# chan0park/node2vec-by-ecc

Hardware: AMD Instinct MI355X
Metric: walk-steps/s (higher is better)
Workload: dtype f64 alias draw / int32 ids (walk); f32 (SGNS)

## Files before the change

### node2vec-by-ecc_amd/csrc/n2v_tables.hip

```cpp
#include "n2v_walk_step.h"
#include "n2v_wave_table.h"

namespace {

using n2v::uni;
using n2v::uni64;

constexpr int kLdsSlots = 512;

struct TabArgs {
    n2v::RowCtx g;
    const int32_t* src_of;
    const int64_t* edge_off;
    const int32_t* order;
    int64_t e_begin, e_end;
    const n2v_edge_rec* recs;
    n2v_alias_slot* thin;
    n2v_fat_slot* fat;
    int32_t* status;
    unsigned long long* work;
    unsigned char* scratch;
    int64_t max_k;
};

constexpr int kChunk = 16;

template <typename Slot>
__device__ __forceinline__ void emit_fat(const TabArgs& a, const Slot* T, int64_t t0, int64_t base, int K, int lane) {
    for (int k = lane; k < K; k += 64) {
        const double q = T[k].q;
        const int J = T[k].J;
        n2v::write_fat_slot(a.fat + t0 + k, q, a.recs + base + k, a.recs + base + J);
    }
}

struct FatEmit {
    const n2v_edge_rec* recs;
    n2v_fat_slot* fat;
    __device__ __forceinline__ void operator()(bool active, int idx, double q, int J) const {
        if (active) n2v::write_fat_slot(fat + idx, q, recs + idx, recs + J);
    }
};
struct ThinEmit {
    n2v_alias_slot* thin;
    __device__ __forceinline__ void operator()(bool active, int idx, double q, int J) const {
        if (!active) return;
        n2v_alias_slot s;
        s.q = q; s.J = J; s.aux = 0;
        thin[idx] = s;
    }
};

template <bool FAT, int RULE>
__global__ void __launch_bounds__(256) edge_tables_wave_kernel(TabArgs a) {
    __shared__ n2v_alias_slot lds[4 * kLdsSlots];
    __shared__ double feed[4 * n2v::kFeed];
    __shared__ int32_t rows[4 * n2v::kRowCache];
    const int lane = threadIdx.x & 63;
    const int wv = __builtin_amdgcn_readfirstlane(threadIdx.x >> 6);
    n2v_alias_slot* Tl = lds + wv * kLdsSlots;
    int32_t* my_row = rows + wv * n2v::kRowCache;
    n2v::WaveScratch ws{feed + wv * n2v::kFeed, my_row, -1};
    int32_t cached_src = -1;
    const int64_t n_waves = (int64_t)gridDim.x * 4;
    bool zero = false;
    unsigned long long nxt = 0, stat = ((unsigned long long)blockIdx.x * 4 + wv) * kChunk;
    auto request_chunk = [&]() {
        if (a.work) { if (lane == 0) nxt = atomicAdd(a.work, (unsigned long long)kChunk); }
        else { nxt = stat; stat += (unsigned long long)n_waves * kChunk; }
    };
    request_chunk();
    for (;;) {
        const int64_t i0 = a.e_begin + uni64((int64_t)nxt);
        if (i0 >= a.e_end) break;
        request_chunk();
        const int n_in = (int)min((int64_t)kChunk, a.e_end - i0);
        int32_t h_src = 0, h_dst = 0, h_K = 0;
        int64_t h_base = 0, h_t0 = 0;
        if (lane < n_in) {
            const int64_t e = a.order ? (int64_t)(uint32_t)a.order[i0 + lane] : i0 + lane;
            h_src = a.src_of[e];
            h_dst = a.g.col[e];
            h_base = a.g.row_ptr[h_dst];
            h_K = (int32_t)(a.g.row_ptr[h_dst + 1] - h_base);
            h_t0 = a.edge_off[e];
        }
      for (int j = 0; j < n_in; ++j) {
        const int32_t src = __builtin_amdgcn_readlane(h_src, j);
        const int K = __builtin_amdgcn_readlane(h_K, j);
        if (K == 0) continue;
        const int64_t base = ((int64_t)__builtin_amdgcn_readlane((int)(h_base >> 32), j) << 32) |
                             (uint32_t)__builtin_amdgcn_readlane((int)h_base, j);
        const int64_t t0 = ((int64_t)__builtin_amdgcn_readlane((int)(h_t0 >> 32), j) << 32) |
                           (uint32_t)__builtin_amdgcn_readlane((int)h_t0, j);
        if (RULE == n2v::kRuleNone && src != cached_src) {
            ws.row_n = n2v::wave_cache_row(a.g, my_row, src, lane);
            cached_src = src;
        }
        if (K <= kLdsSlots) {
            if (!n2v::wave_build_table<RULE>(a.g, Tl, ws, src, base, K, lane)) { zero = true; continue; }
            if (FAT) emit_fat(a, Tl, t0, base, K, lane);
            else for (int k = lane; k < K; k += 64) { n2v_alias_slot s = Tl[k]; s.aux = 0; a.thin[t0 + k] = s; }
            __builtin_amdgcn_wave_barrier();
        } else {
            unsigned char* row = a.scratch + ((int64_t)blockIdx.x * 4 + wv) * a.max_k * 12;
            const n2v::StreamStacks S{reinterpret_cast<int32_t*>(row + a.max_k * 8), reinterpret_cast<double*>(row)};
            int32_t* qi = reinterpret_cast<int32_t*>(Tl);
            bool ok;
            if (FAT) {
                n2v::QueueSink<FatEmit> sink{qi, qi + 128, reinterpret_cast<double*>(qi + 256), FatEmit{a.recs + base, a.fat + t0}, lane};
                ok = n2v::wave_build_stream<RULE>(a.g, S, ws, sink, src, base, K, lane);
            } else {
                n2v::QueueSink<ThinEmit> sink{qi, qi + 128, reinterpret_cast<double*>(qi + 256), ThinEmit{a.thin + t0}, lane};
                ok = n2v::wave_build_stream<RULE>(a.g, S, ws, sink, src, base, K, lane);
            }
            if (!ok) { zero = true; continue; }
            __builtin_amdgcn_wave_barrier();
        }
      }
    }
    if (zero && lane == 0) atomicOr(a.status, RULE == n2v::kRulePop ? N2V_STATUS_ZERO_POP : N2V_STATUS_ZERO_NORM);
}

}

namespace {
constexpr int kWgPerCu = n2v::wg_per_cu(4 * (kLdsSlots * 16 + n2v::kFeed * 8 + n2v::kRowCache * 4));
constexpr int64_t kMaxBlocks = 256 * kWgPerCu;
static_assert(kLdsSlots * 16 >= 2048, "the output queue of the large tables overlays the LDS table slice");
inline int64_t scratch_k(int64_t max_degree) { return max_degree <= kLdsSlots ? 0 : (max_degree + 15) / 16 * 16; }
}

extern "C" int64_t n2v_edge_tables_wave_scratch_bytes(int64_t max_degree) {
    return max_degree < 0 ? -1 : kMaxBlocks * 4 * scratch_k(max_degree) * 12;
}

namespace {
template <int RULE>
int launch_edge_tables(int64_t n_nodes, const int64_t* row_ptr, const int32_t* col, const double* w,
                       const int32_t* src_of, double p, double q, int32_t symmetric,
                       const int64_t* edge_off, const int32_t* order, int64_t e_begin, int64_t e_end,
                       const n2v_edge_rec* recs, n2v_alias_slot* thin, n2v_fat_slot* fat,
                       int32_t* status, uint64_t* work_counter, int64_t max_degree, void* scratch,
                       int64_t scratch_bytes, void* stream) {
    if (n_nodes < 0 || e_begin < 0 || e_end < e_begin || max_degree < 0)
        return n2v::fail(N2V_ERR_INVALID, "n2v_build_edge_tables_wave: bad range [%lld, %lld)", (long long)e_begin, (long long)e_end);
    if (e_end == e_begin) return N2V_OK;
    if (!row_ptr || !col || !src_of || !edge_off || !status)
        return n2v::fail(N2V_ERR_INVALID, "n2v_build_edge_tables_wave: null pointer");
    if ((thin == nullptr) == (fat == nullptr))
        return n2v::fail(N2V_ERR_INVALID, "n2v_build_edge_tables_wave: exactly one of thin / fat output");
    if (fat && !recs) return n2v::fail(N2V_ERR_INVALID, "n2v_build_edge_tables_wave: fat output needs the edge records");
    if (fat && ((uintptr_t)fat & 31) != 0) return n2v::fail(N2V_ERR_INVALID, "n2v_build_edge_tables_wave: fat slots not 32-byte aligned");
    if (!(p == p) || !(q == q)) return n2v::fail(N2V_ERR_INVALID, "n2v_build_edge_tables_wave: p or q is NaN");
    int64_t blocks = (e_end - e_begin + 4 * kChunk - 1) / (4 * kChunk);
    if (blocks > kMaxBlocks) blocks = kMaxBlocks;
    const int64_t need = blocks * 4 * scratch_k(max_degree) * 12;
    if (need > 0 && (!scratch || scratch_bytes < need || ((uintptr_t)scratch & 63) != 0))
        return n2v::fail(N2V_ERR_INVALID, "n2v_build_edge_tables_wave: max degree %lld needs %lld bytes of 64-byte aligned scratch "
                         "for %lld workgroups, got %lld", (long long)max_degree, (long long)need, (long long)blocks, (long long)scratch_bytes);
    TabArgs a{n2v::RowCtx{row_ptr, col, w, p, q, symmetric, nullptr}, src_of, edge_off, order, e_begin, e_end, recs, thin, fat, status,
              reinterpret_cast<unsigned long long*>(work_counter), reinterpret_cast<unsigned char*>(scratch), scratch_k(max_degree)};
    if constexpr (RULE == n2v::kRuleNone) {
        if (fat) {
            hipLaunchKernelGGL((edge_tables_wave_kernel<true, RULE>), dim3((unsigned)blocks), dim3(256), 0, (hipStream_t)stream, a);
            return n2v::check_launch("n2v_build_edge_tables_wave");
        }
    }
    hipLaunchKernelGGL((edge_tables_wave_kernel<false, RULE>), dim3((unsigned)blocks), dim3(256), 0, (hipStream_t)stream, a);
    return n2v::check_launch("n2v_build_edge_tables_wave");
}
}

extern "C" int n2v_build_edge_tables_wave(int64_t n_nodes, const int64_t* row_ptr, const int32_t* col, const double* w,
                                          const int32_t* src_of, double p, double q, int32_t symmetric,
                                          const int64_t* edge_off, const int32_t* order, int64_t e_begin, int64_t e_end,
                                          const n2v_edge_rec* recs, n2v_alias_slot* thin, n2v_fat_slot* fat,
                                          int32_t* status, uint64_t* work_counter, int64_t max_degree, void* scratch,
                                          int64_t scratch_bytes, void* stream) {
    return launch_edge_tables<n2v::kRuleNone>(n_nodes, row_ptr, col, w, src_of, p, q, symmetric, edge_off, order, e_begin, e_end, recs,
                                              thin, fat, status, work_counter, max_degree, scratch, scratch_bytes, stream);
}

extern "C" int n2v_build_edge_tables_wave_pop(int64_t n_nodes, const int64_t* row_ptr, const int32_t* col, const double* w,
                                              const int32_t* src_of, double p, const int64_t* edge_off, const int32_t* order,
                                              int64_t e_begin, int64_t e_end, n2v_alias_slot* thin, int32_t* status,
                                              int64_t max_degree, void* scratch, int64_t scratch_bytes, void* stream) {
    if (!thin) return n2v::fail(N2V_ERR_INVALID, "n2v_build_edge_tables_wave_pop: null output");
    if (p == 0.0) return n2v::fail(N2V_ERR_INVALID, "n2v_build_edge_tables_wave_pop: p must be non-zero");
    return launch_edge_tables<n2v::kRulePop>(n_nodes, row_ptr, col, w, src_of, p, 1.0, 0, edge_off, order, e_begin, e_end, nullptr,
                                             thin, nullptr, status, nullptr, max_degree, scratch, scratch_bytes, stream);
}
```

### node2vec-by-ecc_amd/csrc/n2v_wave_table.h

```cpp
#pragma once
#include "n2v_common.h"

namespace n2v {

__device__ __forceinline__ void wave_sync() {
    __builtin_amdgcn_fence(__ATOMIC_RELEASE, "workgroup");
    __builtin_amdgcn_wave_barrier();
    __builtin_amdgcn_fence(__ATOMIC_ACQUIRE, "workgroup");
}
__device__ __forceinline__ double unid(double v) {
    return __hiloint2double(uni(__double2hiint(v)), uni(__double2loint(v)));
}
__device__ __forceinline__ double readlane_f64(double v, int j) {
    const int lo = __builtin_amdgcn_readlane(__double2loint(v), j);
    const int hi = __builtin_amdgcn_readlane(__double2hiint(v), j);
    return __hiloint2double(hi, lo);
}

struct RowCtx {
    const int64_t* row_ptr;
    const int32_t* col;
    const double* w;
    double p, q;
    int32_t symmetric;
    const uint8_t* plain;
};

enum : int { kRuleNone = 0, kRulePop = 1 };
template <int RULE>
__device__ __forceinline__ bool norm_fails(double norm) {
    return RULE == kRulePop ? (norm == 0.0 || norm != norm) : norm == 0.0;
}

constexpr int kFeed = 64;
constexpr int kRowCache = 384;
struct WaveScratch {
    double* feed;
    const int32_t* row;
    int row_n;
    int plain_row = 0;
};

__device__ __forceinline__ int wave_cache_row(const RowCtx& a, int32_t* ws_row, int32_t src, int lane, int cap = kRowCache) {
    if (src < 0 || !a.symmetric) return -1;
    const int64_t b = uni64(a.row_ptr[src]);
    const int S = uni((int)(a.row_ptr[src + 1] - b));
    if (S > cap) return -1;
    for (int i = lane; i < S; i += 64) ws_row[i] = a.col[b + i];
    wave_sync();
    return S;
}

__device__ __forceinline__ bool lds_row_contains(const int32_t* row, int n, int32_t v) {
    int lo = 0, hi = n;
    while (lo < hi) {
        const int mid = (lo + hi) >> 1;
        if (row[mid] < v) lo = mid + 1;
        else hi = mid;
    }
    return lo < n && row[lo] == v;
}

template <int RULE>
__device__ __forceinline__ double step_weight_of(const RowCtx& a, const WaveScratch& ws, int32_t src, int32_t nb, double wt) {
    if (RULE == kRulePop) {
        if (src < 0 && ws.plain_row) return wt;
        const int64_t pop = a.row_ptr[nb + 1] - a.row_ptr[nb];
        if (pop == 0) return __longlong_as_double(0x7FF8000000000000LL);
        if (src >= 0 && nb == src) return wt / (a.p * (double)pop);
        return wt / (double)pop;
    }
    if (src < 0) return wt;
    if (nb == src) return wt / a.p;
    const bool adj = ws.row_n >= 0 ? lds_row_contains(ws.row, ws.row_n, nb)
                     : a.symmetric ? row_contains(a.row_ptr, a.col, src, nb) : row_contains(a.row_ptr, a.col, nb, src);
    return adj ? wt : wt / a.q;
}
template <int RULE>
__device__ __forceinline__ double step_weight(const RowCtx& a, const WaveScratch& ws, int32_t src, int64_t base, int k) {
    return step_weight_of<RULE>(a, ws, src, a.col[base + k], a.w ? a.w[base + k] : 1.0);
}

__device__ __forceinline__ double wave_sum_in_order(const WaveScratch& ws, double norm, double v, int cnt, int lane) {
    ws.feed[lane] = v;
    wave_sync();
    int j = 0;
    for (; j + 8 <= cnt; j += 8) {
#pragma unroll
        for (int i = 0; i < 8; ++i) norm = norm + ws.feed[j + i];
    }
    for (; j < cnt; ++j) norm = norm + ws.feed[j];
    wave_sync();
    return norm;
}

template <typename Stacks, typename Sink>
__device__ __forceinline__ void wave_pair(const Stacks& S, Sink& out, int K, int ns, int nl, int lane) {
    int mem_s = ns, mem_l = nl;
    int s_pos = 0, s_cnt = 0, l_pos = 0, l_cnt = 0;
    int si = 0, li = 0;
    double sq = 0.0, lq = 0.0;
    bool carried = false;
    int cs_i = 0;
    double cs_q = 0.0;
    for (;;) {
        if (l_pos == l_cnt) {
            if (mem_l == 0) break;
            const int pos = K - mem_l + lane;
            l_cnt = min(64, mem_l);
            if (lane < l_cnt) S.load_large(pos, li, lq);
            mem_l -= l_cnt;
            l_pos = 0;
        }
        const int large = __builtin_amdgcn_readlane(li, l_pos);
        double ql = readlane_f64(lq, l_pos);
        ++l_pos;
        if (carried) {
            out.one(cs_i, cs_q, large);
            carried = false;
            ql = ql + cs_q;
            ql = ql - 1.0;
            if (ql < 1.0) { carried = true; cs_i = large; cs_q = ql; continue; }
        }
        bool dry = false;
        for (;;) {
            if (s_pos == s_cnt) {
                if (mem_s == 0) { dry = true; break; }
                const int pos = mem_s - 1 - lane;
                s_cnt = min(64, mem_s);
                if (lane < s_cnt) S.load_small(pos, si, sq);
                mem_s -= s_cnt;
                s_pos = 0;
            }
            const int first = s_pos;
            int dem;
            {
                const int sq_lo = __double2loint(sq), sq_hi = __double2hiint(sq);
                int pos = uni(s_pos);
                const int cnt = uni(s_cnt);
                asm volatile(
                    "s_nop 3\n\t"
                    "1:\n\t"
                    "v_readlane_b32 vcc_lo, %[qlo], %[pos]\n\t"
                    "v_readlane_b32 vcc_hi, %[qhi], %[pos]\n\t"
                    "s_add_i32 %[pos], %[pos], 1\n\t"
                    "s_nop 0\n\t"
                    "v_add_f64 %[ql], %[ql], vcc\n\t"
                    "v_add_f64 %[ql], %[ql], -1.0\n\t"
                    "v_cmp_gt_f64 vcc, 1.0, %[ql]\n\t"
                    "s_cbranch_vccnz 2f\n\t"
                    "s_cmp_lt_i32 %[pos], %[cnt]\n\t"
                    "s_cbranch_scc1 1b\n\t"
                    "s_mov_b32 %[dem], 0\n\t"
                    "s_branch 3f\n\t"
                    "2:\n\t"
                    "s_mov_b32 %[dem], 1\n\t"
                    "3:\n\t"
                    : [ql] "+v"(ql), [pos] "+s"(pos), [dem] "=s"(dem)
                    : [qlo] "v"(sq_lo), [qhi] "v"(sq_hi), [cnt] "s"(cnt)
                    : "vcc", "scc");
                s_pos = pos;
            }
            const bool demoted = dem != 0;
            out.run(lane >= first && lane < s_pos, si, sq, large);
            if (demoted) { carried = true; cs_i = large; cs_q = ql; break; }
        }
        if (dry) {
            out.one(large, ql, 0);
            break;
        }
    }
    if (carried) out.one(cs_i, cs_q, 0);
    if (Sink::kRest) {
        out.rest(lane >= s_pos && lane < s_cnt, si, sq);
        while (mem_s > 0) {
            const int pos = mem_s - 1 - lane;
            const int cnt = min(64, mem_s);
            if (lane < cnt) S.load_small(pos, si, sq);
            out.rest(lane < cnt, si, sq);
            mem_s -= cnt;
        }
        out.rest(lane >= l_pos && lane < l_cnt, li, lq);
        while (mem_l > 0) {
            const int pos = K - mem_l + lane;
            const int cnt = min(64, mem_l);
            if (lane < cnt) S.load_large(pos, li, lq);
            out.rest(lane < cnt, li, lq);
            mem_l -= cnt;
        }
    }
}

template <typename Slot>
struct AosTable {
    Slot* T;
    __device__ __forceinline__ void load_small(int pos, int& idx, double& q) const { idx = T[pos].aux; q = T[idx].q; }
    __device__ __forceinline__ void load_large(int pos, int& idx, double& q) const { idx = T[pos].aux; q = T[idx].q; }
};
template <typename Slot>
struct AosSink {
    static constexpr bool kRest = false;
    Slot* T;
    int lane;
    __device__ __forceinline__ void run(bool in_run, int idx, double, int J) const { if (in_run) T[idx].J = J; }
    __device__ __forceinline__ void one(int idx, double q, int J) const { if (lane == 0) { T[idx].q = q; T[idx].J = J; } }
    __device__ __forceinline__ void rest(bool, int, double) const {}
};

template <int RULE, typename Slot>
__device__ __forceinline__ bool wave_build_table(const RowCtx& a, Slot* T, const WaveScratch ws, int32_t src, int64_t base,
                                                 int K, int lane) {
    for (int k = lane; k < K; k += 64) T[k].q = step_weight<RULE>(a, ws, src, base, k);
    wave_sync();
    double norm = 0.0;
    for (int c = 0; c < K; c += 64)
        norm = wave_sum_in_order(ws, norm, (c + lane < K) ? T[c + lane].q : 0.0, min(64, K - c), lane);
    norm = unid(norm);
    if (norm_fails<RULE>(norm)) return false;
    const double Kd = (double)K;
    int ns = 0, nl = 0;
    for (int c = 0; c < K; c += 64) {
        const int k = c + lane;
        const bool valid = k < K;
        double qk = 0.0;
        if (valid) {
            qk = Kd * (T[k].q / norm);
            T[k].q = qk;
            T[k].J = 0;
        }
        const bool is_small = valid && (qk < 1.0);
        const unsigned long long ms = __ballot(is_small), ml = __ballot(valid && !is_small);
        const unsigned long long below = (1ULL << lane) - 1ULL;
        if (is_small) T[ns + __popcll(ms & below)].aux = k;
        else if (valid) T[K - (nl + __popcll(ml & below) + 1)].aux = k;
        ns += __popcll(ms);
        nl += __popcll(ml);
    }
    ns = uni(ns);
    nl = uni(nl);
    wave_sync();
    AosSink<Slot> sink{T, lane};
    wave_pair(AosTable<Slot>{T}, sink, K, ns, nl, lane);
    wave_sync();
    return true;
}

template <int RULE, typename Slot>
__device__ __forceinline__ bool wave_weights_and_norm(const RowCtx& a, Slot* T, const WaveScratch ws, int32_t src, int64_t base,
                                                      int K, int lane, double& norm_out) {
    for (int k = lane; k < K; k += 64) T[k].q = step_weight<RULE>(a, ws, src, base, k);
    wave_sync();
    double norm = 0.0;
    for (int c = 0; c < K; c += 64)
        norm = wave_sum_in_order(ws, norm, (c + lane < K) ? T[c + lane].q : 0.0, min(64, K - c), lane);
    norm_out = unid(norm);
    return !norm_fails<RULE>(norm_out);
}
template <typename Slot>
__device__ __forceinline__ void wave_finish_table(Slot* T, int K, double norm, int lane) {
    const double Kd = (double)K;
    int ns = 0, nl = 0;
    for (int c = 0; c < K; c += 64) {
        const int k = c + lane;
        const bool valid = k < K;
        double qk = 0.0;
        if (valid) {
            qk = Kd * (T[k].q / norm);
            T[k].q = qk;
            T[k].J = 0;
        }
        const bool is_small = valid && (qk < 1.0);
        const unsigned long long ms = __ballot(is_small), ml = __ballot(valid && !is_small);
        const unsigned long long below = (1ULL << lane) - 1ULL;
        if (is_small) T[ns + __popcll(ms & below)].aux = k;
        else if (valid) T[K - (nl + __popcll(ml & below) + 1)].aux = k;
        ns += __popcll(ms);
        nl += __popcll(ml);
    }
    ns = uni(ns);
    nl = uni(nl);
    wave_sync();
    AosSink<Slot> sink{T, lane};
    wave_pair(AosTable<Slot>{T}, sink, K, ns, nl, lane);
    wave_sync();
}

struct StagedRow {
    const int32_t* g;
    const int32_t* big;
    int n, stride, n_big;
    __device__ __forceinline__ int find(int32_t v) const {
        int lo = 0, hi = n_big;
        while (lo < hi) {
            const int mid = (lo + hi) >> 1;
            if (big[mid] < v) lo = mid + 1;
            else hi = mid;
        }
        if (lo < n_big && big[lo] == v) return lo * stride;
        if (stride == 1 || lo == 0) return -1;
        const int top = min(lo * stride, n);
        int glo = (lo - 1) * stride + 1, ghi = top;
        while (glo < ghi) {
            const int mid = (glo + ghi) >> 1;
            if (g[mid] < v) glo = mid + 1;
            else ghi = mid;
        }
        return (glo < top && g[glo] == v) ? glo : -1;
    }
    __device__ __forceinline__ bool contains(int32_t v) const { return find(v) >= 0; }
};
__device__ __forceinline__ StagedRow stage_row(const int32_t* __restrict__ g, int n, int32_t* big, int cap, int lane) {
    const int stride = (n + cap - 1) / cap;
    const int n_big = (n + stride - 1) / stride;
    for (int i = lane; i < n_big; i += 64) big[i] = g[(int64_t)i * stride];
    wave_sync();
    return StagedRow{g, big, n, stride, n_big};
}

constexpr int kSpecCap = 128;
struct ClassSweep {
    const int32_t* M;
    int m;
    int smask;
    double qv;
    __device__ __forceinline__ bool sm(int cl) const { return (smask >> cl) & 1; }
    __device__ __forceinline__ double qc(int cl) const { return readlane_f64(qv, uni(cl)); }
};
struct RunIter {
    int j, top;
    int want;
    int r_top, r_cnt, r_cls;
    __device__ __forceinline__ void next(const ClassSweep& c) {
        for (;;) {
            if (top < 0) { r_cnt = 0; return; }
            const int e = j >= 0 ? uni(c.M[j]) : -4;
            const int spos = e >> 2;
            if (spos == top) {
                --j;
                r_top = top; r_cnt = 1; r_cls = e & 3;
                --top;
            } else {
                r_top = top; r_cnt = top - spos; r_cls = 0;
                top = spos;
            }
            if ((int)c.sm(r_cls) == want) return;
        }
    }
    __device__ __forceinline__ void take(const ClassSweep& c, int n) {
        r_top -= n;
        r_cnt -= n;
        if (r_cnt == 0) next(c);
    }
};
__device__ __forceinline__ int dyadic_draw(const RowCtx& a, const WaveScratch& ws, int32_t prev, int64_t base, int K, int kk,
                                           double u2, double wp, double wq, bool exact_sum, int32_t* big, int cap, int32_t* spec,
                                           int lane) {
    if (prev < 0) {
        const double q = (double)K * (1.0 / (double)K);
        return (u2 < q) ? kk : 0;
    }
    const int64_t pb = uni64(a.row_ptr[prev]);
    const int S = uni((int)(a.row_ptr[prev + 1] - pb));
    const int32_t* rc = a.col + base;
    const int32_t* rp = a.col + pb;
    const bool cached = ws.row_n >= 0;
    int n_adj = 0, p_idx = -1;
    const unsigned long long below = (1ULL << lane) - 1ULL;
    auto note = [&](bool adj, int pos) {
        const unsigned long long m = __ballot(adj);
        const int at = n_adj + __popcll(m & below);
        if (adj && at < kSpecCap) spec[at] = pos;
        n_adj += __popcll(m);
    };
    if ((cached && K <= 8 * S) || K <= S) {
        StagedRow R{rp, ws.row, S, 1, S};
        if (!cached) R = stage_row(rp, S, big, cap, lane);
        for (int c = 0; c < K; c += 64) {
            const int k = c + lane;
            bool adj = false, isp = false;
            if (k < K) {
                const int32_t nb = rc[k];
                isp = nb == prev;
                adj = !isp && R.contains(nb);
            }
            note(adj, k);
            const unsigned long long mp = __ballot(isp);
            if (mp != 0ULL) p_idx = c + __builtin_ctzll(mp);
        }
    } else {
        const StagedRow R = stage_row(rc, K, big, cap, lane);
        for (int c = 0; c < S; c += 64) {
            const int i = c + lane;
            int pos = -1;
            if (i < S) {
                const int32_t x = cached ? ws.row[i] : rp[i];
                if (x != prev) pos = R.find(x);
            }
            note(pos >= 0, pos);
        }
        p_idx = R.find(prev);
    }
    n_adj = uni(n_adj);
    p_idx = uni(p_idx);
    wave_sync();
    const int n_prev = p_idx >= 0 ? 1 : 0;
    const int m = n_adj + n_prev;
    if (m > kSpecCap) return -2;
    {
        const int v0 = lane < n_adj ? spec[lane] : 0x3FFFFFFF, v1 = 64 + lane < n_adj ? spec[64 + lane] : 0x3FFFFFFF;
        const int before = __popcll(__ballot(v0 < p_idx)) + __popcll(__ballot(v1 < p_idx));
        wave_sync();
        if (lane < n_adj) spec[lane + ((n_prev && v0 > p_idx) ? 1 : 0)] = v0 * 4 + 1;
        if (64 + lane < n_adj) spec[64 + lane + ((n_prev && v1 > p_idx) ? 1 : 0)] = v1 * 4 + 1;
        if (n_prev && lane == 0) spec[before] = p_idx * 4 + 2;
        wave_sync();
    }
    double norm;
    if (exact_sum) {
        norm = ((double)n_prev * wp + (double)n_adj) + (double)(K - n_prev - n_adj) * wq;
    } else {
        norm = 0.0;
        int pos = 0;
        for (int j = 0; j <= m; ++j) {
            const int e = j < m ? uni(spec[j]) : K * 4;
            for (int g = (e >> 2) - pos; g > 0; --g) norm = norm + wq;
            if (j < m) norm = norm + ((e & 3) == 2 ? wp : 1.0);
            pos = (e >> 2) + 1;
        }
        norm = unid(norm);
    }
    if (norm == 0.0) return -2;
    const double Kd = (double)K;
    const double q0 = Kd * (wq / norm), q1 = Kd * (1.0 / norm), q2 = Kd * (wp / norm);
    const ClassSweep c{spec, m, (q0 < 1.0 ? 1 : 0) | (q1 < 1.0 ? 2 : 0) | (q2 < 1.0 ? 4 : 0),
                       lane == 0 ? q0 : (lane == 1 ? q1 : q2)};
    int cls_kk = 0;
    {
        const int e0 = lane < m ? spec[lane] : -4, e1 = 64 + lane < m ? spec[64 + lane] : -4;
        const unsigned long long h0 = __ballot((e0 >> 2) == kk), h1 = __ballot((e1 >> 2) == kk);
        if (h0) cls_kk = __builtin_amdgcn_readlane(e0, __builtin_ctzll(h0)) & 3;
        else if (h1) cls_kk = __builtin_amdgcn_readlane(e1, __builtin_ctzll(h1)) & 3;
    }
    double q_kk = c.qc(cls_kk);
    if (q_kk < 1.0 && u2 < q_kk) return kk;
    RunIter sm_{m - 1, K - 1, 1, 0, 0, 0}, lg_{m - 1, K - 1, 0, 0, 0, 0};
    sm_.next(c);
    lg_.next(c);
    int J_kk = 0, c_i = 0;
    bool carried = false, done = false;
    double c_q = 0.0;
    while (!done && lg_.r_cnt > 0 && (carried || sm_.r_cnt > 0)) {
        const int large = lg_.r_top;
        double ql = c.qc(lg_.r_cls);
        lg_.take(c, 1);
        for (;;) {
            if (carried) {
                carried = false;
                if (c_i == kk) { J_kk = large; q_kk = c_q; done = true; break; }
                ql = ql + c_q;
                ql = ql - 1.0;
            } else {
                if (sm_.r_cnt == 0) { if (large == kk) q_kk = ql; done = true; break; }
                const double qs = c.qc(sm_.r_cls);
                int n = sm_.r_cnt;
                const bool hit = kk <= sm_.r_top && kk > sm_.r_top - n;
                if (hit) n = sm_.r_top - kk;
                int used = 0;
                bool dem = false;
                while (used < n) {
                    ql = ql + qs;
                    ql = ql - 1.0;
                    ++used;
                    if (uni((int)(ql < 1.0))) { dem = true; break; }
                }
                sm_.take(c, used);
                if (!dem) {
                    if (hit) { J_kk = large; q_kk = qs; done = true; break; }
                    continue;
                }
            }
            if (uni((int)(ql < 1.0))) {
                if (lg_.r_cnt == 0) { if (large == kk) q_kk = ql; done = true; }
                else { carried = true; c_i = large; c_q = ql; }
                break;
            }
        }
    }
    return (u2 < q_kk) ? kk : J_kk;
}

template <int RULE>
__device__ __forceinline__ int wave_draw_le64(const RowCtx& a, const WaveScratch& ws, int32_t src, int64_t base, int32_t nb, int K,
                                              int kk, double u2, bool exact_sum, double wp, double wq, int lane) {
    const bool valid = lane < K;
    double w, norm, w_kk;
    if (RULE == kRuleNone && exact_sum) {
        const bool isp = valid && src >= 0 && nb == src;
        const bool adj = valid && src >= 0 && !isp &&
                         (ws.row_n >= 0 ? lds_row_contains(ws.row, ws.row_n, nb) : row_contains(a.row_ptr, a.col, src, nb));
        const unsigned long long mp = __ballot(isp), ma = __ballot(adj);
        if (src < 0) { norm = (double)K; w_kk = 1.0; w = 1.0; }
        else {
            const int n_prev = __popcll(mp), n_adj = __popcll(ma);
            norm = ((double)n_prev * wp + (double)n_adj) + (double)(K - n_prev - n_adj) * wq;
            w_kk = ((mp >> kk) & 1ULL) ? wp : (((ma >> kk) & 1ULL) ? 1.0 : wq);
            w = isp ? wp : (adj ? 1.0 : wq);
        }
    } else {
        w = valid ? step_weight_of<RULE>(a, ws, src, nb, a.w ? a.w[base + lane] : 1.0) : 0.0;
        norm = unid(wave_sum_in_order(ws, 0.0, w, K, lane));
        if (norm_fails<RULE>(norm)) return -1;
        w_kk = readlane_f64(w, kk);
    }
    double q_kk = (double)K * (w_kk / norm);
    if (q_kk < 1.0 && u2 < q_kk) return kk;
    const double q = valid ? (double)K * (w / norm) : 0.0;
    unsigned long long ms = __ballot(valid && q < 1.0), ml = __ballot(valid && !(q < 1.0));
    int J_kk = 0;
    bool carried = false, done = false;
    int c_i = 0;
    double c_q = 0.0;
    while (!done && ml != 0ULL && (carried || ms != 0ULL)) {
        const int large = 63 - __builtin_clzll(ml);
        ml &= ~(1ULL << large);
        double ql = readlane_f64(q, large);
        for (;;) {
            int small;
            double qs;
            if (carried) { small = c_i; qs = c_q; carried = false; }
            else if (ms != 0ULL) { small = 63 - __builtin_clzll(ms); ms &= ~(1ULL << small); qs = readlane_f64(q, small); }
            else {
                if (large == kk) q_kk = ql;
                done = true;
                break;
            }
            if (small == kk) { J_kk = large; q_kk = qs; done = true; break; }
            ql = ql + qs;
            ql = ql - 1.0;
            if (uni((int)(ql < 1.0))) {
                if (ml == 0ULL) { if (large == kk) q_kk = ql; done = true; }
                else { carried = true; c_i = large; c_q = ql; }
                break;
            }
            if (large == kk && ms == 0ULL) { q_kk = ql; done = true; break; }
        }
    }
    return (u2 < q_kk) ? kk : J_kk;
}

struct StreamStacks {
    int32_t* idx;
    double* q;
    __device__ __forceinline__ void load_small(int pos, int& i, double& v) const { i = idx[pos]; v = q[pos]; }
    __device__ __forceinline__ void load_large(int pos, int& i, double& v) const { i = idx[pos]; v = q[pos]; }
};

template <typename Emit>
struct QueueSink {
    static constexpr bool kRest = true;
    int32_t* qi;
    int32_t* qJ;
    double* qq;
    Emit emit;
    int lane;
    int n = 0;
    __device__ __forceinline__ void flush64() {
        wave_sync();
        emit(true, qi[lane], qq[lane], qJ[lane]);
        wave_sync();
        const int rem = n - 64;
        if (lane < rem) { const int i = qi[64 + lane], J = qJ[64 + lane]; const double q = qq[64 + lane];
                          qi[lane] = i; qJ[lane] = J; qq[lane] = q; }
        n = rem;
    }
    __device__ __forceinline__ void run(bool in_run, int idx, double q, int J) {
        const unsigned long long m = __ballot(in_run);
        if (in_run) { const int p = n + __popcll(m & ((1ULL << lane) - 1ULL)); qi[p] = idx; qJ[p] = J; qq[p] = q; }
        n += __popcll(m);
        if (n >= 64) flush64();
    }
    __device__ __forceinline__ void one(int idx, double q, int J) {
        if (lane == 0) { qi[n] = idx; qJ[n] = J; qq[n] = q; }
        if (++n >= 64) flush64();
    }
    __device__ __forceinline__ void rest(bool in, int idx, double q) { run(in, idx, q, 0); }
    __device__ __forceinline__ void finish() {
        wave_sync();
        emit(lane < n, qi[lane], qq[lane], qJ[lane]);
        n = 0;
        wave_sync();
    }
};

template <int RULE, typename Emit>
__device__ __forceinline__ bool wave_build_stream(const RowCtx& a, const StreamStacks S, const WaveScratch ws,
                                                  QueueSink<Emit>& sink, int32_t src, int64_t base, int K, int lane) {
    double norm = 0.0;
    for (int c = 0; c < K; c += 64)
        norm = wave_sum_in_order(ws, norm, (c + lane < K) ? step_weight<RULE>(a, ws, src, base, c + lane) : 0.0, min(64, K - c), lane);
    norm = unid(norm);
    if (norm_fails<RULE>(norm)) return false;
    const double Kd = (double)K;
    int ns = 0, nl = 0;
    for (int c = 0; c < K; c += 64) {
        const int k = c + lane;
        const bool valid = k < K;
        double qk = 0.0;
        if (valid) qk = Kd * (step_weight<RULE>(a, ws, src, base, k) / norm);
        const bool is_small = valid && (qk < 1.0);
        const unsigned long long ms = __ballot(is_small), ml = __ballot(valid && !is_small);
        const unsigned long long below = (1ULL << lane) - 1ULL;
        if (valid) {
            const int pos = is_small ? ns + __popcll(ms & below) : K - (nl + __popcll(ml & below) + 1);
            S.idx[pos] = k;
            S.q[pos] = qk;
        }
        ns += __popcll(ms);
        nl += __popcll(ml);
    }
    ns = uni(ns);
    nl = uni(nl);
    wave_sync();
    wave_pair(S, sink, K, ns, nl, lane);
    sink.finish();
    return true;
}

}
```

Measured before the change: 43.79 billion.

## Store LDS alias tables as SoA with halfword indices and overlay row cache

Replaces the per-wave AoS alias slot table in LDS with a structure-of-arrays layout: f64 q plus 16-bit J and aux arrays. The source-row cache now sits inside the tail of the same window instead of a separate LDS array, and is skipped when the table is large enough to overlap it. Together these cut LDS per workgroup from 16 to 12 bytes per slot and drop the row cache, so more workgroups can fit per CU. It also adds a guard and status flag for degrees above max_k, and risks extra row reloads and bank conflicts on the halfword arrays.

```diff
diff --git a/node2vec-by-ecc_amd/csrc/n2v_tables.hip b/node2vec-by-ecc_amd/csrc/n2v_tables.hip
--- a/node2vec-by-ecc_amd/csrc/n2v_tables.hip
+++ b/node2vec-by-ecc_amd/csrc/n2v_tables.hip
@@ -7,6 +7,11 @@
 using n2v::uni64;
 
 constexpr int kLdsSlots = 512;
+constexpr int kTabRow = 384;
+constexpr int kRowFree = kLdsSlots - kTabRow / 2;
+constexpr int kLdsPerWg = 4 * (kLdsSlots * 12 + n2v::kFeed * 8);
+static_assert(kLdsSlots <= 65536 && kTabRow % 2 == 0, "J and the stack words of the LDS window are halfwords");
+static_assert(kRowFree * 8 >= 2048, "the output queue of the large tables overlays the front of the window, before the source row");
 
 struct TabArgs {
     n2v::RowCtx g;
@@ -25,11 +30,12 @@
 
 constexpr int kChunk = 16;
 
-template <typename Slot>
-__device__ __forceinline__ void emit_fat(const TabArgs& a, const Slot* T, int64_t t0, int64_t base, int K, int lane) {
+constexpr int kStatusOverMaxDegree = 4;
+
+__device__ __forceinline__ void emit_fat(const TabArgs& a, const n2v::SoaTable T, int64_t t0, int64_t base, int K, int lane) {
     for (int k = lane; k < K; k += 64) {
-        const double q = T[k].q;
-        const int J = T[k].J;
+        const double q = T.q[k];
+        const int J = T.J[k];
         n2v::write_fat_slot(a.fat + t0 + k, q, a.recs + base + k, a.recs + base + J);
     }
 }
@@ -53,17 +59,17 @@
 
 template <bool FAT, int RULE>
 __global__ void __launch_bounds__(256) edge_tables_wave_kernel(TabArgs a) {
-    __shared__ n2v_alias_slot lds[4 * kLdsSlots];
+    __shared__ double lds_q[4 * kLdsSlots];
+    __shared__ uint16_t lds_J[4 * kLdsSlots], lds_aux[4 * kLdsSlots];
     __shared__ double feed[4 * n2v::kFeed];
-    __shared__ int32_t rows[4 * n2v::kRowCache];
     const int lane = threadIdx.x & 63;
     const int wv = __builtin_amdgcn_readfirstlane(threadIdx.x >> 6);
-    n2v_alias_slot* Tl = lds + wv * kLdsSlots;
-    int32_t* my_row = rows + wv * n2v::kRowCache;
+    const n2v::SoaTable Tl{lds_q + wv * kLdsSlots, lds_J + wv * kLdsSlots, lds_aux + wv * kLdsSlots};
+    int32_t* my_row = reinterpret_cast<int32_t*>(Tl.q + kLdsSlots) - kTabRow;
     n2v::WaveScratch ws{feed + wv * n2v::kFeed, my_row, -1};
     int32_t cached_src = -1;
     const int64_t n_waves = (int64_t)gridDim.x * 4;
-    bool zero = false;
+    bool zero = false, over = false;
     unsigned long long nxt = 0, stat = ((unsigned long long)blockIdx.x * 4 + wv) * kChunk;
     auto request_chunk = [&]() {
         if (a.work) { if (lane == 0) nxt = atomicAdd(a.work, (unsigned long long)kChunk); }
@@ -93,19 +99,25 @@
                              (uint32_t)__builtin_amdgcn_readlane((int)h_base, j);
         const int64_t t0 = ((int64_t)__builtin_amdgcn_readlane((int)(h_t0 >> 32), j) << 32) |
                            (uint32_t)__builtin_amdgcn_readlane((int)h_t0, j);
-        if (RULE == n2v::kRuleNone && src != cached_src) {
-            ws.row_n = n2v::wave_cache_row(a.g, my_row, src, lane);
-            cached_src = src;
+        if (RULE == n2v::kRuleNone) {
+            if (K > kRowFree && K <= kLdsSlots) {
+                ws.row_n = -1;
+                cached_src = -1;
+            } else if (src != cached_src) {
+                ws.row_n = n2v::wave_cache_row(a.g, my_row, src, lane, kTabRow);
+                cached_src = src;
+            }
         }
         if (K <= kLdsSlots) {
             if (!n2v::wave_build_table<RULE>(a.g, Tl, ws, src, base, K, lane)) { zero = true; continue; }
             if (FAT) emit_fat(a, Tl, t0, base, K, lane);
-            else for (int k = lane; k < K; k += 64) { n2v_alias_slot s = Tl[k]; s.aux = 0; a.thin[t0 + k] = s; }
+            else for (int k = lane; k < K; k += 64) { n2v_alias_slot s; s.q = Tl.q[k]; s.J = Tl.J[k]; s.aux = 0; a.thin[t0 + k] = s; }
             __builtin_amdgcn_wave_barrier();
         } else {
+            if (K > a.max_k) { over = true; continue; }
             unsigned char* row = a.scratch + ((int64_t)blockIdx.x * 4 + wv) * a.max_k * 12;
             const n2v::StreamStacks S{reinterpret_cast<int32_t*>(row + a.max_k * 8), reinterpret_cast<double*>(row)};
-            int32_t* qi = reinterpret_cast<int32_t*>(Tl);
+            int32_t* qi = reinterpret_cast<int32_t*>(Tl.q);
             bool ok;
             if (FAT) {
                 n2v::QueueSink<FatEmit> sink{qi, qi + 128, reinterpret_cast<double*>(qi + 256), FatEmit{a.recs + base, a.fat + t0}, lane};
@@ -120,14 +132,14 @@
       }
     }
     if (zero && lane == 0) atomicOr(a.status, RULE == n2v::kRulePop ? N2V_STATUS_ZERO_POP : N2V_STATUS_ZERO_NORM);
+    if (over && lane == 0) atomicOr(a.status, kStatusOverMaxDegree);
 }
 
 }
 
 namespace {
-constexpr int kWgPerCu = n2v::wg_per_cu(4 * (kLdsSlots * 16 + n2v::kFeed * 8 + n2v::kRowCache * 4));
+constexpr int kWgPerCu = n2v::wg_per_cu(kLdsPerWg);
 constexpr int64_t kMaxBlocks = 256 * kWgPerCu;
-static_assert(kLdsSlots * 16 >= 2048, "the output queue of the large tables overlays the LDS table slice");
 inline int64_t scratch_k(int64_t max_degree) { return max_degree <= kLdsSlots ? 0 : (max_degree + 15) / 16 * 16; }
 }
 
diff --git a/node2vec-by-ecc_amd/csrc/n2v_wave_table.h b/node2vec-by-ecc_amd/csrc/n2v_wave_table.h
--- a/node2vec-by-ecc_amd/csrc/n2v_wave_table.h
+++ b/node2vec-by-ecc_amd/csrc/n2v_wave_table.h
@@ -241,6 +241,59 @@
     wave_sync();
     AosSink<Slot> sink{T, lane};
     wave_pair(AosTable<Slot>{T}, sink, K, ns, nl, lane);
+    wave_sync();
+    return true;
+}
+
+struct SoaTable {
+    double* q;
+    uint16_t* J;
+    uint16_t* aux;
+    __device__ __forceinline__ void load_small(int pos, int& idx, double& v) const { idx = aux[pos]; v = q[idx]; }
+    __device__ __forceinline__ void load_large(int pos, int& idx, double& v) const { idx = aux[pos]; v = q[idx]; }
+};
+struct SoaSink {
+    static constexpr bool kRest = false;
+    SoaTable T;
+    int lane;
+    __device__ __forceinline__ void run(bool in_run, int idx, double, int J) const { if (in_run) T.J[idx] = (uint16_t)J; }
+    __device__ __forceinline__ void one(int idx, double q, int J) const { if (lane == 0) { T.q[idx] = q; T.J[idx] = (uint16_t)J; } }
+    __device__ __forceinline__ void rest(bool, int, double) const {}
+};
+template <int RULE>
+__device__ __forceinline__ bool wave_build_table(const RowCtx& a, const SoaTable T, const WaveScratch ws, int32_t src, int64_t base,
+                                                 int K, int lane) {
+    for (int k = lane; k < K; k += 64) T.q[k] = step_weight<RULE>(a, ws, src, base, k);
+    wave_sync();
+    double norm = 0.0;
+    for (int c = 0; c < K; c += 64)
+        norm = wave_sum_in_order(ws, norm, (c + lane < K) ? T.q[c + lane] : 0.0, min(64, K - c), lane);
+    norm = unid(norm);
+    if (norm_fails<RULE>(norm)) return false;
+    const double Kd = (double)K;
+    int ns = 0, nl = 0;
+    for (int c = 0; c < K; c += 64) {
+        const int k = c + lane;
+        const bool valid = k < K;
+        double qk = 0.0;
+        if (valid) {
+            qk = Kd * (T.q[k] / norm);
+            T.q[k] = qk;
+            T.J[k] = 0;
+        }
+        const bool is_small = valid && (qk < 1.0);
+        const unsigned long long ms = __ballot(is_small), ml = __ballot(valid && !is_small);
+        const unsigned long long below = (1ULL << lane) - 1ULL;
+        if (is_small) T.aux[ns + __popcll(ms & below)] = (uint16_t)k;
+        else if (valid) T.aux[K - (nl + __popcll(ml & below) + 1)] = (uint16_t)k;
+        ns += __popcll(ms);
+        nl += __popcll(ml);
+    }
+    ns = uni(ns);
+    nl = uni(nl);
+    wave_sync();
+    SoaSink sink{T, lane};
+    wave_pair(T, sink, K, ns, nl, lane);
     wave_sync();
     return true;
 }
```

Measured after the change: 43.20 billion. -1.3%, worse.
